# jhauret/vibravox

Measured on AMD Instinct MI355X. Metric: EBEN train-step audio-seconds/sec (gen+disc), higher is better.
Workload: dtype bf16

## Files before the change

vibravox_amd/csrc/gen_conv.hip:

```cpp
#include "common.h"

#include <cstdlib>
#include <type_traits>

namespace eben {

typedef float f32x16 __attribute__((ext_vector_type(16)));
typedef float f32x2 __attribute__((ext_vector_type(2)));
typedef __bf16 bf16x8 __attribute__((ext_vector_type(8)));
typedef __bf16 bf16x2 __attribute__((ext_vector_type(2)));
typedef unsigned u32x4 __attribute__((ext_vector_type(4)));

struct GcArgs {
  const float* x; float* y; const u32x4* wp; const float* bias; const float* res;
  int B, CX, LX, CY, LY, NU, S;
  int rpc_shift, off0, KSP, nkg;
  int nrt, nrg, ncb, nh;
  int reflect;
  float in_slope, out_slope, res_slope;
  long long w_rt, w_half;
  unsigned xq, xr;
};

__device__ __forceinline__ unsigned gc_pack2(float a, float b) {
// ... 267 lines not shown
        __syncthreads();
      }
    };
    for (int ch = 0; ch + 1 < nch; ++ch) chunk(ch, std::true_type{});
    chunk(nch - 1, std::false_type{});
  };
  bool allfast = true;
#pragma unroll
  for (int ct = 0; ct < CT; ++ct) allfast = allfast && fast[ct];
  if (allfast) {
    if (act_in) run(std::true_type{}, std::true_type{});
    else run(std::true_type{}, std::false_type{});
  } else {
    if (act_in) run(std::false_type{}, std::true_type{});
    else run(std::false_type{}, std::false_type{});
  }

  if (EBEN_GC_DBG & 8) {
    float s = 0.f;
#pragma unroll
    for (int ct = 0; ct < CT; ++ct)
#pragma unroll
      for (int i = 0; i < RT; ++i)
#pragma unroll
        for (int r = 0; r < 16; ++r) s += acc[ct][i][r];
    if (s == 1.2345f) P.y[0] = s;
    return;
  }
  float* yb = P.y + (long long)b * P.CY * P.LY;
  const float* rb = P.res ? P.res + (long long)b * P.CY * P.LY : nullptr;
#pragma unroll
  for (int ct = 0; ct < CT; ++ct) {
    const int u = u0w + ct * 32 + n;
    if (u >= P.NU) continue;
#pragma unroll
    for (int i = 0; i < RT; ++i) {
      const int mt = (rg * RT + i) * 32;
#pragma unroll
      for (int r4 = 0; r4 < 4; ++r4) {
        const int m = mt + 8 * r4 + 4 * hk;
        float o[4];
#pragma unroll
        for (int r = 0; r < 4; ++r) o[r] = acc[ct][i][4 * r4 + r];
        if (FORM != 2) {
#pragma unroll
          for (int r = 0; r < 4; ++r) {
            const float t = o[r] + (P.bias ? P.bias[m + r] : 0.f);
            const long long yi = (long long)(m + r) * P.LY + u;
            yb[yi] = lrelu(t, P.out_slope) + (rb ? lrelu(rb[yi], P.res_slope) : 0.f);
          }
        } else if (P.S == 8) {
          const int co = m >> 2;
          const float bv = P.bias ? P.bias[co] : 0.f;
          f32x4 t;
#pragma unroll
          for (int r = 0; r < 4; ++r) t[r] = lrelu(o[r] + bv, P.out_slope);
          const long long yi = (long long)co * P.LY + 8 * u + 4 * h;
          if (rb) {
            const f32x4 rv = *reinterpret_cast<const f32x4*>(rb + yi);
#pragma unroll
            for (int r = 0; r < 4; ++r) t[r] += lrelu(rv[r], P.res_slope);
          }
          *reinterpret_cast<f32x4*>(yb + yi) = t;
        } else if (P.S == 4) {
#pragma unroll
          for (int c2 = 0; c2 < 2; ++c2) {
            const int co = (m >> 1) + c2;
            const float bv = P.bias ? P.bias[co] : 0.f;
            f32x2 t;
            t[0] = lrelu(o[2 * c2] + bv, P.out_slope); t[1] = lrelu(o[2 * c2 + 1] + bv, P.out_slope);
            const long long yi = (long long)co * P.LY + 4 * u + 2 * h;
            if (rb) { t[0] += lrelu(rb[yi], P.res_slope); t[1] += lrelu(rb[yi + 1], P.res_slope); }
            *reinterpret_cast<f32x2*>(yb + yi) = t;
          }
        } else {
#pragma unroll
          for (int r = 0; r < 4; ++r) {
            const float t = o[r] + (P.bias ? P.bias[m + r] : 0.f);
            const long long yi = (long long)(m + r) * P.LY + 2 * u + h;
            yb[yi] = lrelu(t, P.out_slope) + (rb ? lrelu(rb[yi], P.res_slope) : 0.f);
          }
        }
      }
    }
  }
}

struct GcPackArgs {
  const float* w; const float* scale; u32x4* wp;
  int form, CX, CY, k, S, pad, rpc_shift, nkg, KSP, nrt, nh, np;
  long long total;
};

__global__ __launch_bounds__(256) void gc_pack_kernel(const GcPackArgs P) {
  const long long i = (long long)blockIdx.x * 256 + threadIdx.x;
  if (i >= P.total) return;
  const int lane = (int)(i & 63);
  long long r = i >> 6;
  const int q = (int)(r % P.np); r /= P.np;
  const int ks = (int)(r % P.KSP); r /= P.KSP;
  const int rt = (int)(r % P.nrt);
  const int h = (int)(r / P.nrt);
  const int mr = rt * 32 + (lane & 31);
  const int kg = 2 * ks + (lane >> 5);
  float v[8];
#pragma unroll
  for (int e = 0; e < 8; ++e) {
    float t = 0.f;
    if (kg < P.nkg) {
      if (P.form != 2) {
        const int chan = P.form == 0 ? kg >> P.rpc_shift : 2 * kg + (e >> 2);
        const int j = P.form == 0 ? 8 * (kg & ((1 << P.rpc_shift) - 1)) + e : (e & 3);
        if (j < P.k && chan < P.CX && mr < P.CY)
          t = P.w[((long long)mr * P.CX + chan) * P.k + j] * (P.scale ? P.scale[mr] : 1.f);
      } else {
        const int chan = 4 * kg + (e >> 1);
        const int hs = P.S >> 1;
        const int co = mr / hs, p = h * hs + mr % hs;
        const int du = h == 0 ? 1 - (e & 1) : -(e & 1);
        const int j = P.S * du + p + P.pad;
        if (j >= 0 && j < P.k && chan < P.CX && co < P.CY)
          t = P.w[((long long)chan * P.CY + co) * P.k + j] * (P.scale ? P.scale[chan] : 1.f);
      }
    }
    v[e] = t;
  }
  u32x4 o;
  for (int qq = 0;; ++qq) {
    o[0] = gc_pack2(v[0], v[1]); o[1] = gc_pack2(v[2], v[3]); o[2] = gc_pack2(v[4], v[5]); o[3] = gc_pack2(v[6], v[7]);
    if (qq == q) break;
#pragma unroll
    for (int u = 0; u < 4; ++u) {
      v[2 * u] -= __builtin_bit_cast(float, o[u] << 16);
      v[2 * u + 1] -= __builtin_bit_cast(float, o[u] & 0xffff0000u);
    }
  }
  P.wp[i] = o;
}

static int gc_env(const char* name, int dflt) {
  const char* s = getenv(name);
  return s ? atoi(s) : dflt;
}

struct GcPlan {
  int ok, form, np;
  int CX, LX, CY, LY, NU, S, k, pad, rpc_shift, nkg, KSP, rows, nrt, nh;
  int RT, CT, nrg, ncb;
};

static void gc_plan(const Canon& c, int dir, GcPlan* p) {
  static const int enabled = gc_env("EBEN_GC", 1);
  memset(p, 0, sizeof(*p));
  if (!enabled || c.bl || (c.np != 3 && c.np != 2) || c.g != 1 || c.d != 1 || c.xsplit_dir >= 0) return;
  p->np = c.np;
  p->S = c.s; p->k = c.k;
  if (dir == 0) {
    const bool enc = c.k == 2 * c.s && (c.s == 2 || c.s == 4 || c.s == 8);
    const bool lat = c.s == 1 && c.k >= 5 && c.k <= 8;
    if (!(enc || lat) || c.Cin % 16 || c.Cout % 32) return;
    if (c.reflect && (c.pl > c.Lin - 1 || c.pr > c.Lin - 1)) return;
    p->form = c.k <= 4 ? 1 : 0;
    p->CX = c.Cin; p->LX = c.Lin; p->CY = c.Cout; p->LY = c.Lout; p->NU = c.Lout;
    p->pad = c.pl;
    p->rpc_shift = c.k > 8 ? 1 : 0;
    p->nkg = p->form == 0 ? c.Cin << p->rpc_shift : c.Cin / 2;
    p->rows = c.Cout; p->nh = 1;
  } else {
    if (c.s != 2 && c.s != 4 && c.s != 8) return;
    if (c.k != 2 * c.s || c.pl != c.s / 2 || c.Lin != c.s * c.Lout) return;
    if (c.Cout % 16 || (c.Cin * (c.s / 2)) % 32) return;
    p->form = 2;
    p->CX = c.Cout; p->LX = c.Lout; p->CY = c.Cin; p->LY = c.Lin; p->NU = c.Lout;
    p->pad = c.pl;
    p->nkg = c.Cout / 4;
    p->rows = c.Cin * (c.s / 2); p->nh = 2;
  }
  p->KSP = round_up(ceil_div(p->nkg, 2), 8);
  p->nrt = p->rows / 32;
  static const int env_rt = gc_env("EBEN_GC_RT", 0), env_ct = gc_env("EBEN_GC_CT", 0);
  double best = 1e30;
  const int prod = p->np == 3 ? 6 : p->np == 2 ? 3 : 1;
  for (int rt : {2, 1}) {
    if (p->nrt % rt) continue;
    for (int ct : {2, 1}) {
      if (rt == 1 && ct == 2) continue;
      if ((env_rt && rt != env_rt && p->nrt % env_rt == 0) || (env_ct && ct != env_ct)) continue;
      const int ncb = ceil_div(p->NU, 128 * ct);
      const long long waves = 4ll * p->nh * (p->nrt / rt) * c.B * ncb;
      const double per_wave = (double)p->KSP * ct * (32.0 * prod * rt > 240.0 ? 32.0 * prod * rt : 240.0) + 2500.0 + 600.0 * rt * ct;
      const double t = (double)((waves + 1023) / 1024) * per_wave * (ct == 2 ? 1.05 : 1.0);
      if (t < best * 0.98) { best = t; p->RT = rt; p->CT = ct; }
    }
  }
  if (!p->RT) return;
  p->nrg = p->nrt / p->RT;
  p->ncb = ceil_div(p->NU, 128 * p->CT);
  p->ok = 1;
}

int gc_applicable(const Canon& c, int dir) {
  GcPlan p;
  gc_plan(c, dir, &p);
  return p.ok;
}

size_t gc_packed_floats(const Canon& c, int dir) {
  GcPlan p;
  gc_plan(c, dir, &p);
  return p.ok ? (size_t)p.nh * p.nrt * p.KSP * p.np * 64 * 4 : 0;
}

int gc_pack(const Canon& c, int dir, const float* w, const float* scale, float* wp, hipStream_t st) {
  GcPlan p;
  gc_plan(c, dir, &p);
  if (!p.ok) return fail(EBEN_EUNSUPPORTED, "gc_pack on a layer the direct-operand conv does not cover");
  GcPackArgs a{};
  a.w = w; a.scale = scale; a.wp = reinterpret_cast<u32x4*>(wp);
  a.form = p.form; a.CX = p.CX; a.CY = p.CY; a.k = p.k; a.S = p.S; a.pad = p.pad; a.rpc_shift = p.rpc_shift; a.nkg = p.nkg; a.KSP = p.KSP;
  a.nrt = p.nrt; a.nh = p.nh; a.np = p.np;
  a.total = (long long)p.nh * p.nrt * p.KSP * p.np * 64;
  hipLaunchKernelGGL(gc_pack_kernel, dim3((unsigned)((a.total + 255) / 256)), dim3(256), 0, st, a);
  EBEN_CHECK_LAUNCH("gc_pack_kernel");
  return EBEN_OK;
}

template <int FORM, int NP>
static void gc_launch_shape(const GcPlan& p, const GcArgs& a, unsigned grid, hipStream_t st) {
  if (p.RT == 2 && p.CT == 2) hipLaunchKernelGGL((gc_kernel<FORM, 2, 2, NP>), dim3(grid), dim3(256), 0, st, a);
  else if (p.RT == 2) hipLaunchKernelGGL((gc_kernel<FORM, 2, 1, NP>), dim3(grid), dim3(256), 0, st, a);
  else hipLaunchKernelGGL((gc_kernel<FORM, 1, 1, NP>), dim3(grid), dim3(256), 0, st, a);
}

int gc_launch(const Canon& c, int dir, const TapIO& io, hipStream_t st) {
  GcPlan p;
  gc_plan(c, dir, &p);
  if (!p.ok) return fail(EBEN_EUNSUPPORTED, "gc_launch on a layer the direct-operand conv does not cover");
  if (io.emask || io.in_mode || io.accumulate || io.res_rows || io.fm_sums) return fail(EBEN_EUNSUPPORTED, "direct-operand conv: forward launches only");
  GcArgs a{};
  a.x = io.x; a.y = io.y; a.wp = reinterpret_cast<const u32x4*>(io.wp); a.bias = io.bias; a.res = io.res;
  a.B = c.B; a.CX = p.CX; a.LX = p.LX; a.CY = p.CY; a.LY = p.LY; a.NU = p.NU; a.S = p.S;
  a.rpc_shift = p.rpc_shift; a.off0 = -p.pad; a.KSP = p.KSP; a.nkg = p.nkg;
  a.nrt = p.nrt; a.nrg = p.nrg; a.ncb = p.ncb; a.nh = p.nh;
  a.reflect = dir == 0 ? c.reflect : 0;
  a.in_slope = io.in_slope; a.out_slope = io.out_slope; a.res_slope = io.res_slope;
  a.w_rt = (long long)p.KSP * p.np * 64; a.w_half = a.w_rt * p.nrt;
  const unsigned grid = (unsigned)(p.nh * p.nrg * c.B * p.ncb);
  a.xq = grid / 8; a.xr = grid % 8;
  if (p.np == 2) {
    if (p.form == 0) gc_launch_shape<0, 2>(p, a, grid, st);
    else if (p.form == 1) gc_launch_shape<1, 2>(p, a, grid, st);
    else gc_launch_shape<2, 2>(p, a, grid, st);
  } else if (p.form == 0) gc_launch_shape<0, 3>(p, a, grid, st);
  else if (p.form == 1) gc_launch_shape<1, 3>(p, a, grid, st);
  else gc_launch_shape<2, 3>(p, a, grid, st);
  EBEN_CHECK_LAUNCH("gc_kernel");
  return EBEN_OK;
}

}
```

vibravox_amd/csrc/ru_split.hip:

```cpp
#include "common.h"

#include <cstdlib>

namespace eben {

#ifndef EBEN_RU_DBG
#define EBEN_RU_DBG 0
#endif

typedef float f32x16 __attribute__((ext_vector_type(16)));
typedef float f32x2 __attribute__((ext_vector_type(2)));
typedef __bf16 bf16x8 __attribute__((ext_vector_type(8)));
typedef __bf16 bf16x2 __attribute__((ext_vector_type(2)));
typedef unsigned u32x4 __attribute__((ext_vector_type(4)));

__device__ __forceinline__ unsigned rs_pack_bf16(float a, float b) {
  const f32x2 v = {a, b};
  return __builtin_bit_cast(unsigned, __builtin_convertvector(v, bf16x2));
}

template <int NP>
__device__ __forceinline__ void rs_split8(const float (&v)[8], u32x4 (&p)[NP]) {
  float r[8];
#pragma unroll
// ... 170 lines not shown
        for (int q = 0; q < 4; ++q) {
          uint2 v;
          v.x = rs_pack_bf16(acc1[i][4 * q], acc1[i][4 * q + 1]);
          v.y = rs_pack_bf16(acc1[i][4 * q + 2], acc1[i][4 * q + 3]);
          if (!(EBEN_RU_DBG & 2) || v.x == 0x12345u) hu[(long long)(4 * i + q) * L * 2] = v;
        }
    }
  } else if (P.h != nullptr && live) {
    float* __restrict__ hb = P.h + lbase;
#pragma unroll
    for (int i = 0; i < CT; ++i)
#pragma unroll
      for (int r = 0; r < 16; ++r) {
        const unsigned m = i * 32 + (r & 3) + 8 * (r >> 2) + 4 * (lane >> 5);
        hb[m * (unsigned)L] = acc1[i][r];
      }
  }

#pragma unroll
  for (int c2 = 0; c2 < NCH2; ++c2) {
    const int ch = NCH1 + c2;
    if (ch + 1 < NCHK) issue_w(ch + 1);
    const u32x4* wb = Ws + (ch & 1) * WCHU + lane;
#pragma unroll
    for (int kk = 0; kk < KSC; ++kk) {
      const int ks2 = c2 * KSC + kk;
      const int isrc = ks2 >> 1, s = ks2 & 1;
      float v[8];
#pragma unroll
      for (int e = 0; e < 8; ++e) v[e] = acc1[isrc][8 * s + e];
      u32x4 a[NP][CT], bq[NP];
#pragma unroll
      for (int q = 0; q < NP; ++q)
#pragma unroll
        for (int i = 0; i < CT; ++i) a[q][i] = wb[kk * U + (q * CT + i) * 64];
      rs_split8<NP>(v, bq);
      rs_mma<NP, CT>(a, bq, acc2);
    }
    if (c2 + 1 < NCH2) __syncthreads();
  }

  if constexpr (BL) {
    unsigned nlo = 0, nhi = 0;
#pragma unroll
    for (int i = 0; i < CT; ++i)
#pragma unroll
      for (int q = 0; q < 4; ++q) {
        unsigned nib = 0;
#pragma unroll
        for (int e = 0; e < 4; ++e) nib |= (acc2[i][4 * q + e] > 0.f ? 1u : 0u) << e;
        if (i < 2) nlo |= nib << (4 * (4 * i + q));
        else nhi |= nib << (4 * (4 * (i - 2) + q));
      }
    const unsigned olo = __shfl_xor(nlo, 32, 64), ohi = CT > 2 ? __shfl_xor(nhi, 32, 64) : 0u;
    const int hf = lane >> 5;
    const unsigned l0 = hf ? olo : nlo, l1 = hf ? nlo : olo, h0 = hf ? ohi : nhi, h1 = hf ? nhi : ohi;
    if (live) {
      unsigned char* __restrict__ ub8 = P.um + ubase;
#pragma unroll
      for (int g = 0; g < 4 * CT; g += 2) {
        const int gg = g + hf;
        const unsigned w0 = gg < 8 ? l0 : h0, w1 = gg < 8 ? l1 : h1;
        const int sh = 4 * (gg & 7);
        ub8[(long long)gg * L] = (unsigned char)(((w0 >> sh) & 15u) | (((w1 >> sh) & 15u) << 4));
      }
    }
  }

  if (!live) return;
  const float* xc = Xs + xshift + d + col;
  float* __restrict__ yb = P.y + lbase;
  float* __restrict__ ub = P.u + lbase;
  const bool keep_u = !BL && P.u != nullptr;
#pragma unroll
  for (int i = 0; i < CT; ++i)
#pragma unroll
    for (int r = 0; r < 16; ++r) {
      const unsigned m = i * 32 + (r & 3) + 8 * (r >> 2) + 4 * (lane >> 5);
      const unsigned off = m * (unsigned)L;
      const float uu = lrelu(acc2[i][r], P.out_slope);
      if (keep_u) ub[off] = uu;
      if (!(EBEN_RU_DBG & 1) || uu == 12345.f) yb[off] = xc[m * XS] + uu;
    }
}

__device__ __forceinline__ void ru3_pack_fwd_body(const float* __restrict__ vd, const float* __restrict__ sd, const float* __restrict__ vp,
                                                  const float* __restrict__ sp, u32x4* __restrict__ img, int CT, int NP, unsigned bid, unsigned nblk) {
  const int C = 32 * CT, KB = C / 16;
  const int total = 4 * KB * CT * 64;
  for (int t = bid * 256 + threadIdx.x; t < total; t += nblk * 256) {
    const int lane = t & 63;
    const int i = (t >> 6) % CT;
    const int ks = t / (64 * CT);
    const int m = 32 * i + (lane & 31), kh = lane >> 5;
    float w[8];
    if (ks < 3 * KB) {
      const int j = ks / KB, cb = ks - j * KB;
#pragma unroll
      for (int e = 0; e < 8; ++e) w[e] = vd[((long long)m * C + cb * 16 + 8 * kh + e) * 3 + j] * (sd ? sd[m] : 1.f);
    } else {
      const int ks2 = ks - 3 * KB, isrc = ks2 >> 1, s = ks2 & 1;
#pragma unroll
      for (int e = 0; e < 8; ++e) {
        const int chn = 32 * isrc + (e & 3) + 8 * (2 * s + (e >> 2)) + 4 * kh;
        w[e] = vp[(long long)m * C + chn] * (sp ? sp[m] : 1.f);
      }
    }
    float r[8];
#pragma unroll
    for (int e = 0; e < 8; ++e) r[e] = w[e];
    for (int q = 0; q < NP; ++q) {
      u32x4 o;
#pragma unroll
      for (int e = 0; e < 4; ++e) o[e] = rs_pack_bf16(r[2 * e], r[2 * e + 1]);
      img[((long long)(ks * NP + q) * CT + i) * 64 + lane] = o;
#pragma unroll
      for (int e = 0; e < 4; ++e) {
        r[2 * e] -= __builtin_bit_cast(float, o[e] << 16);
        r[2 * e + 1] -= __builtin_bit_cast(float, o[e] & 0xffff0000u);
      }
    }
  }
}

struct Ru3BwdArgs {
  const float* gy; const float* u; const u32x4* wimg; const float* xmask; const float* post; float* gx; float* gh;
  int B, L, d, ntt, BO, vec;
  float out_slope, in_slope;
};

template <int CT, int NW, int NP, int G>
__global__ __launch_bounds__(NW * 64, (NW == 4 && CT < 4) ? 2 : 1) void ru3_bwd_kernel(const Ru3BwdArgs P) {
  constexpr int NT = NW * 64, WN = NW * 32, C = 32 * CT;
  constexpr int GS = WN + 4;
  constexpr int U = NP * CT * 64;
  constexpr int EU = 2 * U;
  constexpr int WCHU = G * EU;
  static_assert(CT % G == 0, "an entry group never straddles a stage");

  extern __shared__ __attribute__((aligned(16))) u32x4 rs_smem[];
  u32x4* Ws = rs_smem;
  float* Gs = reinterpret_cast<float*>(rs_smem + 2 * WCHU);

  const int tid = threadIdx.x, lane = tid & 63;
  const int wn = __builtin_amdgcn_readfirstlane(tid >> 6);
  const int tt = __builtin_amdgcn_readfirstlane(blockIdx.x % P.ntt);
  const int b = __builtin_amdgcn_readfirstlane(blockIdx.x / P.ntt);
  const int d = P.d, L = P.L, BO = P.BO;
  const int t0 = tt * BO;
  const int w0 = t0 - d;
  const int wa = w0 >= 0 ? (w0 & ~3) : w0;
  const int xshift = w0 - wa;
  const long long rowbase = (long long)b * C * L;

  const bool fold_l = t0 <= d && L > 1;
  const bool fold_r = t0 + BO > L - 1 - d && t0 <= L - 2;
  const int NS = 4 * CT + (fold_l ? CT : 0) + (fold_r ? CT : 0);
  const int NSG = NS / G;
  auto img_entry = [&](int sq) -> int {
    if (sq < 4 * CT) return sq;
    sq -= 4 * CT;
    if (fold_l) { if (sq < CT) return CT + 2 * CT + sq; sq -= CT; }
    return CT + sq;
  };
  auto issue_w = [&](int sg) {
    u32x4* dst = Ws + (sg & 1) * WCHU;
// ... 182 lines not shown

__device__ __forceinline__ void ru3_pack_bwd_body(const float* __restrict__ vd, const float* __restrict__ sd, const float* __restrict__ vp,
                                                  const float* __restrict__ sp, u32x4* __restrict__ img, int CT, int NP, unsigned bid, unsigned nblk) {
  const int C = 32 * CT;
  const int total = 4 * CT * 2 * CT * 64;
  for (int t = bid * 256 + threadIdx.x; t < total; t += nblk * 256) {
    const int lane = t & 63;
    const int i = (t >> 6) % CT;
    const int kk = (t / (64 * CT)) & 1;
    const int en = t / (128 * CT);
    const int row = 32 * i + (lane & 31), kh = lane >> 5;
    float w[8];
#pragma unroll
    for (int e = 0; e < 8; ++e) {
      if (en < CT) {
        const int m = en * 32 + kk * 16 + 8 * kh + e;
        w[e] = vp[(long long)m * C + row] * (sp ? sp[m] : 1.f);
      } else {
        const int jj = (en - CT) / CT, cb = (en - CT) - jj * CT;
        const int m = cb * 32 + kk * 16 + 8 * kh + e;
        w[e] = vd[((long long)m * C + row) * 3 + (2 - jj)] * (sd ? sd[m] : 1.f);
      }
    }
    float r[8];
#pragma unroll
    for (int e = 0; e < 8; ++e) r[e] = w[e];
    for (int q = 0; q < NP; ++q) {
      u32x4 o;
#pragma unroll
      for (int e = 0; e < 4; ++e) o[e] = rs_pack_bf16(r[2 * e], r[2 * e + 1]);
      img[(((long long)(en * 2 + kk) * NP + q) * CT + i) * 64 + lane] = o;
#pragma unroll
      for (int e = 0; e < 4; ++e) {
        r[2 * e] -= __builtin_bit_cast(float, o[e] << 16);
        r[2 * e + 1] -= __builtin_bit_cast(float, o[e] & 0xffff0000u);
      }
    }
  }
}

__global__ __launch_bounds__(256) void ru3_pack_fwd_kernel(const float* vd, const float* sd, const float* vp, const float* sp, u32x4* img, int CT, int NP) {
  ru3_pack_fwd_body(vd, sd, vp, sp, img, CT, NP, blockIdx.x, gridDim.x);
}
__global__ __launch_bounds__(256) void ru3_pack_bwd_kernel(const float* vd, const float* sd, const float* vp, const float* sp, u32x4* img, int CT, int NP) {
  ru3_pack_bwd_body(vd, sd, vp, sp, img, CT, NP, blockIdx.x, gridDim.x);
}

constexpr int RU_PACK_MULTI = 48;
struct RuPackTable {
  int n;
  unsigned short first[RU_PACK_MULTI + 1];
  struct { const float* vd; const float* sd; const float* vp; const float* sp; u32x4* img; short CT, NP, which, pad; } job[RU_PACK_MULTI];
};
__global__ __launch_bounds__(256) void ru3_pack_multi_kernel(const RuPackTable T) {
  int j = 0;
#pragma unroll 1
  while (j + 1 < T.n && blockIdx.x >= T.first[j + 1]) ++j;
  const unsigned bid = blockIdx.x - T.first[j], nblk = T.first[j + 1] - T.first[j];
  if (T.job[j].which == 0) ru3_pack_fwd_body(T.job[j].vd, T.job[j].sd, T.job[j].vp, T.job[j].sp, T.job[j].img, T.job[j].CT, T.job[j].NP, bid, nblk);
  else ru3_pack_bwd_body(T.job[j].vd, T.job[j].sd, T.job[j].vp, T.job[j].sp, T.job[j].img, T.job[j].CT, T.job[j].NP, bid, nblk);
}

static int rs_pieces(int math) {
  switch (math) {
    case EBEN_MATH_BF16: return 1;
    case EBEN_MATH_BF16X3: return 2;
    case EBEN_MATH_BF16X6: return 3;
    default: return 0;
  }
}

template <int CT, int NW, int NP, int KSC, bool BL = false>
static int launch_ru3_fwd(const Ru3Args& a, hipStream_t st) {
  static LdsAttrOnce attr_once;
  auto kern = ru3_fwd_kernel<CT, NW, NP, KSC, BL>;
  constexpr int XS = NW * 32 + 2 * RS_DMAX + 6;
  const size_t lds = (size_t)2 * KSC * NP * CT * 64 * 16 + sizeof(float) * 32 * CT * XS;
  {
    const hipError_t e = lds_attr_once(attr_once, reinterpret_cast<const void*>(kern));
    if (e != hipSuccess) return hip_fail(e, "hipFuncSetAttribute(ru3_fwd)");
  }
  hipLaunchKernelGGL(kern, dim3(a.B * a.ntt), dim3(NW * 64), lds, st, a);
  EBEN_CHECK_LAUNCH("ru3_fwd_kernel");
  return EBEN_OK;
}

template <int CT, int NW, int NP, int G>
static int launch_ru3_bwd(const Ru3BwdArgs& a, hipStream_t st) {
  static LdsAttrOnce attr_once;
  auto kern = ru3_bwd_kernel<CT, NW, NP, G>;
  constexpr int GS = NW * 32 + 4;
  const size_t lds = (size_t)2 * G * 2 * NP * CT * 64 * 16 + sizeof(float) * 32 * CT * GS;
  {
    const hipError_t e = lds_attr_once(attr_once, reinterpret_cast<const void*>(kern));
    if (e != hipSuccess) return hip_fail(e, "hipFuncSetAttribute(ru3_bwd)");
  }
  hipLaunchKernelGGL(kern, dim3(a.B * a.ntt), dim3(NW * 64), lds, st, a);
  EBEN_CHECK_LAUNCH("ru3_bwd_kernel");
  return EBEN_OK;
}

static int rs_waves(int channels) {
  static const int w128 = getenv("EBEN_RU3_W128") ? atoi(getenv("EBEN_RU3_W128")) : 4;
  return channels == 128 ? (w128 == 4 ? 4 : 2) : 4;
}

int ru3_supported(int channels, int dilation, int math) {
  return (channels == 32 || channels == 64 || channels == 128) && dilation >= 1 && dilation <= RS_DMAX && rs_pieces(math) > 0;
}

size_t ru3_packed_floats(int channels, int math) {
  const int np = rs_pieces(math);
  if (np == 0 || (channels != 32 && channels != 64 && channels != 128)) return 0;
  return (size_t)2 * np * channels * channels;
}

int ru3_pack(int channels, int math, int which, const float* vd, const float* sd, const float* vp, const float* sp, float* wimg, hipStream_t st) {
  const int np = rs_pieces(math), CT = channels / 32;
  const int total = which == 0 ? 8 * CT * CT * 64 : 4 * CT * 2 * CT * 64;
  if (which == 0)
    hipLaunchKernelGGL(ru3_pack_fwd_kernel, dim3(ceil_div(total, 256)), dim3(256), 0, st, vd, sd, vp, sp, reinterpret_cast<u32x4*>(wimg), CT, np);
  else
    hipLaunchKernelGGL(ru3_pack_bwd_kernel, dim3(ceil_div(total, 256)), dim3(256), 0, st, vd, sd, vp, sp, reinterpret_cast<u32x4*>(wimg), CT, np);
  EBEN_CHECK_LAUNCH("ru3_pack_kernel");
  return EBEN_OK;
}

int ru3_fwd(int math, int batch, int channels, int length, int dilation, const float* x, float in_slope, float out_slope, const float* wimg,
            float* y, float* h, float* u, hipStream_t st) {
  Ru3Args a;
  a.x = x; a.wimg = reinterpret_cast<const u32x4*>(wimg); a.y = y; a.h = h; a.u = u;
  a.xb = nullptr; a.hb = nullptr; a.um = nullptr;
  a.B = batch; a.L = length; a.d = dilation;
  const int bn = rs_waves(channels) * 32;
  a.ntt = ceil_div(length, bn);
  a.in_slope = in_slope; a.out_slope = out_slope;
  a.vec = ((reinterpret_cast<uintptr_t>(x) & 15) == 0 && (length & 3) == 0) ? 1 : 0;
  if ((long long)a.B * a.ntt > 0x7fffffffLL) return fail(EBEN_EINVAL, "ResidualUnit grid too large");
  const int np = rs_pieces(math);
#define EBEN_RU3_FWD(NPV)                                                 \
  switch (channels / 32) {                                                \
    case 1: return launch_ru3_fwd<1, 4, NPV, 2>(a, st);                   \
    case 2: return launch_ru3_fwd<2, 4, NPV, 2>(a, st);                   \
    default: return rs_waves(128) == 4 ? launch_ru3_fwd<4, 4, NPV, 2>(a, st) : launch_ru3_fwd<4, 2, NPV, 1>(a, st); \
  }
  switch (np) {
    case 1: EBEN_RU3_FWD(1)
    case 2: EBEN_RU3_FWD(2)
    default: EBEN_RU3_FWD(3)
  }
#undef EBEN_RU3_FWD
}

int ru3_fwd_bl(int math, int batch, int channels, int length, int dilation, const float* x, float in_slope, float out_slope, const float* wimg,
               float* y, void* xb, void* hb, void* um, hipStream_t st) {
  Ru3Args a;
  a.x = x; a.wimg = reinterpret_cast<const u32x4*>(wimg); a.y = y; a.h = nullptr; a.u = nullptr;
  a.xb = static_cast<u32x4*>(xb); a.hb = static_cast<u32x4*>(hb); a.um = static_cast<unsigned char*>(um);
  a.B = batch; a.L = length; a.d = dilation;
  a.ntt = ceil_div(length, 128);
  a.in_slope = in_slope; a.out_slope = out_slope;
  a.vec = ((reinterpret_cast<uintptr_t>(x) & 15) == 0 && (length & 3) == 0) ? 1 : 0;
  if ((long long)a.B * a.ntt > 0x7fffffffLL) return fail(EBEN_EINVAL, "ResidualUnit grid too large");
  const int np = rs_pieces(math);
  if (np != 3 && np != 2) return fail(EBEN_EUNSUPPORTED, "eben_rubl_fwd: the forward computes in EBEN_MATH_BF16X6 or EBEN_MATH_BF16X3 (got %d)", math);
  if (np == 2) {
    switch (channels / 32) {
      case 1: return launch_ru3_fwd<1, 4, 2, 2, true>(a, st);
      case 2: return launch_ru3_fwd<2, 4, 2, 2, true>(a, st);
      default: return launch_ru3_fwd<4, 4, 2, 2, true>(a, st);
    }
  }
  switch (channels / 32) {
    case 1: return launch_ru3_fwd<1, 4, 3, 2, true>(a, st);
    case 2: return launch_ru3_fwd<2, 4, 3, 2, true>(a, st);
    default: return launch_ru3_fwd<4, 4, 3, 2, true>(a, st);
  }
}

int ru3_bwd(int math, int batch, int channels, int length, int dilation, const float* gy, const float* u, float out_slope, const float* x,
            float in_slope, const float* post, const float* wimg, float* gx, float* gh, hipStream_t st) {
  Ru3BwdArgs a;
  a.gy = gy; a.u = u; a.wimg = reinterpret_cast<const u32x4*>(wimg); a.xmask = in_slope != 1.f ? x : nullptr; a.post = post; a.gx = gx; a.gh = gh;
  a.B = batch; a.L = length; a.d = dilation;
  const int nw = rs_waves(channels);
  const int wn = nw * 32;
  a.BO = wn - 2 * dilation; a.ntt = ceil_div(length, a.BO);
  a.out_slope = out_slope; a.in_slope = in_slope;
  a.vec = (((reinterpret_cast<uintptr_t>(gy) | reinterpret_cast<uintptr_t>(u)) & 15) == 0 && (length & 3) == 0) ? 1 : 0;
  if ((long long)a.B * a.ntt > 0x7fffffffLL) return fail(EBEN_EINVAL, "ResidualUnit grid too large");
  const int np = rs_pieces(math);
  switch (np) {
    case 1:
      switch (channels / 32) {
        case 1: return launch_ru3_bwd<1, 4, 1, 1>(a, st);
        case 2: return launch_ru3_bwd<2, 4, 1, 2>(a, st);
        default: return nw == 4 ? launch_ru3_bwd<4, 4, 1, 2>(a, st) : launch_ru3_bwd<4, 2, 1, 2>(a, st);
      }
    case 2:
      switch (channels / 32) {
        case 1: return launch_ru3_bwd<1, 4, 2, 1>(a, st);
        case 2: return launch_ru3_bwd<2, 4, 2, 2>(a, st);
        default: return rs_waves(128) == 4 ? launch_ru3_bwd<4, 4, 2, 1>(a, st) : launch_ru3_bwd<4, 2, 2, 1>(a, st);
      }
    default:
      switch (channels / 32) {
        case 1: return launch_ru3_bwd<1, 4, 3, 1>(a, st);
        case 2: return launch_ru3_bwd<2, 4, 3, 1>(a, st);
        default: return rs_waves(128) == 4 ? launch_ru3_bwd<4, 4, 3, 1>(a, st) : launch_ru3_bwd<4, 2, 3, 1>(a, st);
      }
  }
}

}

using namespace eben;

extern "C" size_t eben_ru_packed_floats_ex(int channels, int math) {
  if (math == EBEN_MATH_F32) return eben_ru_packed_floats(channels);
  return ru3_packed_floats(channels, math);
}

extern "C" int eben_ru_supported(int channels, int dilation, int math) {
  if (math == EBEN_MATH_F32) return (channels == 32 || channels == 64 || channels == 128) && dilation >= 1 && dilation <= 16;
  return ru3_supported(channels, dilation, math);
}

extern "C" int eben_ru_pack_ex(int channels, int math, int which, const float* v_dil, const float* scale_dil, const float* v_pw,
                               const float* scale_pw, float* wimg, void* stream) {
  EBEN_REQUIRE(which == 0 || which == 1, "ru_pack_ex: which = 0 (forward image) or 1 (backward image)");
  if (math == EBEN_MATH_F32)
    return which == 0 ? eben_ru_pack(channels, v_dil, scale_dil, v_pw, scale_pw, wimg, stream)
                      : eben_ru_pack_bwd(channels, v_dil, scale_dil, v_pw, scale_pw, wimg, stream);
  EBEN_REQUIRE(ru3_supported(channels, 1, math), "fused ResidualUnit: 32, 64 or 128 channels and a known math mode (got %d, %d)", channels, math);
  EBEN_REQUIRE(v_dil && v_pw && wimg, "null pointer in ru_pack_ex");
  return ru3_pack(channels, math, which, v_dil, scale_dil, v_pw, scale_pw, wimg, as_stream(stream));
}

extern "C" int eben_ru_pack_multi(const EbenRuPackJob* jobs, int n, void* stream) {
  EBEN_REQUIRE(n >= 0 && (n == 0 || jobs != nullptr), "bad ru pack job list");
  for (int base = 0; base < n; base += RU_PACK_MULTI) {
    RuPackTable T;
    T.n = n - base < RU_PACK_MULTI ? n - base : RU_PACK_MULTI;
    T.first[0] = 0;
    for (int j = 0; j < T.n; ++j) {
      const EbenRuPackJob& jb = jobs[base + j];
      EBEN_REQUIRE(jb.math != EBEN_MATH_F32, "ru_pack_multi: the split-operand images only (pack the fp32 MFMA images with eben_ru_pack)");
      EBEN_REQUIRE(ru3_supported(jb.channels, 1, jb.math) && (jb.which == 0 || jb.which == 1) && jb.v_dil && jb.v_pw && jb.wimg, "bad ru pack job %d", base + j);
// ... 42 lines not shown
```

Before: 7437.

## Add split-K gen conv kernel for small grids and presplit RU forward

Adds a split-K variant of the direct-operand generator conv. When the grid would be small (short outputs, deep K), four waves each take a quarter of the K steps and their partial sums are reduced through LDS, giving more blocks and waves on the GPU. It also adds a residual-unit forward kernel for the 2-piece bf16 path that splits the input into bf16 pieces once while staging it in LDS, so the split is not repeated per k-step. Both are on by default, with the presplit kernel limited to 128+ channels unless the env var is set to 2. The cost is extra LDS traffic, a block-level reduction and more code paths.

```diff
diff --git a/vibravox_amd/csrc/gen_conv.hip b/vibravox_amd/csrc/gen_conv.hip
--- a/vibravox_amd/csrc/gen_conv.hip
+++ b/vibravox_amd/csrc/gen_conv.hip
@@ -373,6 +373,160 @@
           }
         }
       }
+    }
+  }
+}
+
+template <int RT, int NP>
+__global__ __launch_bounds__(256, 2) void gc_ks_kernel(const GcArgs P) {
+  constexpr int KD = 4;
+  __shared__ __attribute__((aligned(16))) float Rs[4 * RT * 16 * 64];
+
+  const int tid = threadIdx.x;
+  const int lane = tid & 63;
+  const int wave = __builtin_amdgcn_readfirstlane(tid >> 6);
+  const int n = lane & 31, hk = lane >> 5;
+
+  unsigned id;
+  {
+    const unsigned bid = blockIdx.x, xcd = bid & 7u, idx = bid >> 3;
+    id = (xcd < P.xr ? xcd * (P.xq + 1) : P.xr * (P.xq + 1) + (xcd - P.xr) * P.xq) + idx;
+  }
+  const int rg = __builtin_amdgcn_readfirstlane((int)(id % (unsigned)P.nrg)); id /= (unsigned)P.nrg;
+  const int cb = __builtin_amdgcn_readfirstlane((int)(id % (unsigned)P.ncb));
+  const int b = __builtin_amdgcn_readfirstlane((int)(id / (unsigned)P.ncb));
+
+  const float* xb = P.x + (long long)b * P.CX * P.LX;
+  const u32x4* wsrc = P.wp + (long long)(rg * RT) * P.w_rt;
+  const int nk = P.KSP >> 2, ks0 = wave * nk;
+
+  typedef const __attribute__((address_space(1))) char* gptr_t;
+  const int u0 = cb * 32;
+  const int ucol = u0 + n < P.NU ? u0 + n : P.NU - 1;
+  const bool fast = u0 + 31 < P.NU && P.S * u0 + P.off0 >= 0 && P.S * (u0 + 31) + P.off0 + (8 << P.rpc_shift) <= P.LX;
+  const bool act_in = P.in_slope != 1.f;
+  const int ks_real = P.nkg >> 1;
+  const int RKS = P.rpc_shift ? 1 : 2;
+  const int loff = (P.rpc_shift ? 8 * hk : hk * P.LX) + P.S * ucol + P.off0;
+  auto row_ptr = [&](int ks) -> gptr_t {
+    const int kc = ks < ks_real ? ks : ks_real - 1;
+    unsigned long long a = reinterpret_cast<unsigned long long>(xb + (long long)(kc * RKS) * P.LX);
+    asm volatile("" : "+s"(a));
+    return reinterpret_cast<gptr_t>(a);
+  };
+  auto w_ptr = [&](int ks) -> gptr_t {
+    unsigned long long a = reinterpret_cast<unsigned long long>(wsrc + (long long)ks * (NP * 64));
+    asm volatile("" : "+s"(a));
+    return reinterpret_cast<gptr_t>(a);
+  };
+  struct Slow { int off[8]; unsigned ok; };
+  Slow sl;
+  if (!fast) {
+    sl.ok = 0;
+#pragma unroll
+    for (int e = 0; e < 8; ++e) {
+      const int crow = P.rpc_shift ? 0 : hk;
+      int pos = P.S * ucol + P.off0 + (P.rpc_shift ? 8 * hk : 0) + e;
+      if (P.reflect) {
+        pos = pos < 0 ? -pos : pos;
+        pos = pos >= P.LX ? 2 * (P.LX - 1) - pos : pos;
+      }
+      const bool ok = pos >= 0 && pos < P.LX;
+      sl.off[e] = crow * P.LX + (ok ? pos : 0);
+      sl.ok |= (unsigned)ok << e;
+    }
+  }
+
+  f32x16 acc[RT];
+#pragma unroll
+  for (int i = 0; i < RT; ++i)
+#pragma unroll
+    for (int r = 0; r < 16; ++r) acc[i][r] = 0.f;
+
+  auto run = [&](auto fast_tag, auto act_tag) {
+    constexpr bool FAST = decltype(fast_tag)::value;
+    float v[KD][8];
+    u32x4 aq[KD][NP][RT];
+    typedef float f4u __attribute__((ext_vector_type(4), aligned(4)));
+    typedef const __attribute__((address_space(1))) f4u* g4_t;
+    typedef const __attribute__((address_space(1))) float* g1_t;
+    typedef const __attribute__((address_space(1))) u32x4* gu_t;
+    auto ask = [&](int k, int s) {
+      const int ks = ks0 + (k < nk ? k : nk - 1);
+      const gptr_t rp = row_ptr(ks);
+      if constexpr (FAST) {
+        const unsigned o = (unsigned)loff * 4u;
+        const f4u a0 = *reinterpret_cast<g4_t>(rp + o), a1 = *reinterpret_cast<g4_t>(rp + 16 + o);
+#pragma unroll
+        for (int e = 0; e < 4; ++e) { v[s][e] = a0[e]; v[s][4 + e] = a1[e]; }
+      } else {
+#pragma unroll
+        for (int e = 0; e < 8; ++e) v[s][e] = *reinterpret_cast<g1_t>(rp + (unsigned)sl.off[e] * 4u);
+      }
+      const gptr_t wq = w_ptr(ks);
+#pragma unroll
+      for (int q = 0; q < NP; ++q)
+#pragma unroll
+        for (int i = 0; i < RT; ++i)
+          aq[s][q][i] = *reinterpret_cast<gu_t>(wq + ((unsigned)i * (unsigned)P.w_rt + (unsigned)(q * 64 + lane)) * 16u);
+    };
+#pragma unroll
+    for (int s = 0; s < KD; ++s) ask(s, s);
+    for (int k = 0; k < nk; k += KD) {
+#pragma unroll
+      for (int s = 0; s < KD; ++s) {
+        if constexpr (!FAST) {
+#pragma unroll
+          for (int e = 0; e < 8; ++e) v[s][e] = (sl.ok >> e) & 1u ? v[s][e] : 0.f;
+        }
+        if constexpr (decltype(act_tag)::value) {
+#pragma unroll
+          for (int e = 0; e < 8; ++e) v[s][e] = lrelu(v[s][e], P.in_slope);
+        }
+        u32x4 bq[NP];
+        gc_split<NP>(v[s], bq);
+#pragma unroll
+        for (int lvl = NP - 1; lvl >= 0; --lvl)
+#pragma unroll
+          for (int qw = 0; qw < NP; ++qw) {
+            const int qx = lvl - qw;
+            if (qx < 0 || qx >= NP) continue;
+#pragma unroll
+            for (int i = 0; i < RT; ++i)
+              acc[i] = __builtin_amdgcn_mfma_f32_32x32x16_bf16(__builtin_bit_cast(bf16x8, aq[s][qw][i]), __builtin_bit_cast(bf16x8, bq[qx]), acc[i], 0, 0, 0);
+          }
+        ask(k + s + KD, s);
+        __builtin_amdgcn_sched_barrier(0);
+      }
+    }
+  };
+  if (fast) {
+    if (act_in) run(std::true_type{}, std::true_type{});
+    else run(std::true_type{}, std::false_type{});
+  } else {
+    if (act_in) run(std::false_type{}, std::true_type{});
+    else run(std::false_type{}, std::false_type{});
+  }
+
+#pragma unroll
+  for (int i = 0; i < RT; ++i)
+#pragma unroll
+    for (int r = 0; r < 16; ++r) Rs[((wave * RT + i) * 16 + r) * 64 + lane] = acc[i][r];
+  __syncthreads();
+  const int u = u0 + n;
+  if (u >= P.NU) return;
+  float* yb = P.y + (long long)b * P.CY * P.LY;
+  const float* rb = P.res ? P.res + (long long)b * P.CY * P.LY : nullptr;
+#pragma unroll
+  for (int i = 0; i < RT; ++i) {
+    const int m = (rg * RT + i) * 32 + 8 * wave + 4 * hk;
+#pragma unroll
+    for (int r = 0; r < 4; ++r) {
+      const int ri = (i * 16 + 4 * wave + r) * 64 + lane;
+      const float o = (Rs[ri] + Rs[RT * 1024 + ri]) + (Rs[2 * RT * 1024 + ri] + Rs[3 * RT * 1024 + ri]);
+      const float t = o + (P.bias ? P.bias[m + r] : 0.f);
+      const long long yi = (long long)(m + r) * P.LY + u;
+      yb[yi] = lrelu(t, P.out_slope) + (rb ? lrelu(rb[yi], P.res_slope) : 0.f);
     }
   }
 }
@@ -438,6 +592,7 @@
   int ok, form, np;
   int CX, LX, CY, LY, NU, S, k, pad, rpc_shift, nkg, KSP, rows, nrt, nh;
   int RT, CT, nrg, ncb;
+  int ksplit;
 };
 
 static void gc_plan(const Canon& c, int dir, GcPlan* p) {
@@ -488,6 +643,21 @@
   p->nrg = p->nrt / p->RT;
   p->ncb = ceil_div(p->NU, 128 * p->CT);
   p->ok = 1;
+  static const int ksplit = gc_env("EBEN_GC_KSPLIT", 1);
+  if (ksplit && p->form == 0 && p->NU <= 128 && p->KSP >= 64 && p->KSP % 16 == 0 && (long long)p->nh * p->nrg * c.B * p->ncb < 128) {
+    const int ncb = ceil_div(p->NU, 32);
+    double bt = 1e30;
+    int brt = 0;
+    for (int rt : {2, 1}) {
+      if (p->nrt % rt) continue;
+      const long long waves = 4ll * (p->nrt / rt) * c.B * ncb;
+      const double per_wave = (double)(p->KSP / 4) * (32.0 * prod * rt > 240.0 ? 32.0 * prod * rt : 240.0) + 2500.0 + 600.0 * rt;
+      const double t = (double)((waves + 1023) / 1024) * per_wave;
+      if (t < bt * 0.98) { bt = t; brt = rt; }
+    }
+    p->ksplit = 1; p->RT = brt; p->CT = 1;
+    p->nrg = p->nrt / brt; p->ncb = ncb;
+  }
 }
 
 int gc_applicable(const Canon& c, int dir) {
@@ -538,6 +708,15 @@
   a.w_rt = (long long)p.KSP * p.np * 64; a.w_half = a.w_rt * p.nrt;
   const unsigned grid = (unsigned)(p.nh * p.nrg * c.B * p.ncb);
   a.xq = grid / 8; a.xr = grid % 8;
+  if (p.ksplit) {
+    if (p.np == 2) {
+      if (p.RT == 2) hipLaunchKernelGGL((gc_ks_kernel<2, 2>), dim3(grid), dim3(256), 0, st, a);
+      else hipLaunchKernelGGL((gc_ks_kernel<1, 2>), dim3(grid), dim3(256), 0, st, a);
+    } else if (p.RT == 2) hipLaunchKernelGGL((gc_ks_kernel<2, 3>), dim3(grid), dim3(256), 0, st, a);
+    else hipLaunchKernelGGL((gc_ks_kernel<1, 3>), dim3(grid), dim3(256), 0, st, a);
+    EBEN_CHECK_LAUNCH("gc_ks_kernel");
+    return EBEN_OK;
+  }
   if (p.np == 2) {
     if (p.form == 0) gc_launch_shape<0, 2>(p, a, grid, st);
     else if (p.form == 1) gc_launch_shape<1, 2>(p, a, grid, st);
diff --git a/vibravox_amd/csrc/ru_split.hip b/vibravox_amd/csrc/ru_split.hip
--- a/vibravox_amd/csrc/ru_split.hip
+++ b/vibravox_amd/csrc/ru_split.hip
@@ -276,6 +276,228 @@
       if (keep_u) ub[off] = uu;
       if (!(EBEN_RU_DBG & 1) || uu == 12345.f) yb[off] = xc[m * XS] + uu;
     }
+}
+
+template <int CT, int KSC>
+__global__ __launch_bounds__(256, CT < 4 ? 2 : 1) void ru3_fwd_ps_kernel(const Ru3Args P) {
+  constexpr int NP = 2, NT = 256, BN = 128, C = 32 * CT;
+  constexpr int XS = BN + 2 * RS_DMAX + 6;
+  constexpr int PS = (C / 8) * XS;
+  constexpr int KB = C / 16;
+  constexpr int KS1 = 3 * KB, KS2 = KB;
+  constexpr int U = NP * CT * 64;
+  constexpr int WCHU = KSC * U;
+  constexpr int NCH1 = KS1 / KSC, NCH2 = KS2 / KSC, NCHK = NCH1 + NCH2;
+  static_assert(KS1 % KSC == 0 && KS2 % KSC == 0, "a chunk never straddles the two stages");
+  static_assert(KSC % 2 == 0, "the fragment registers alternate by k-step and start every chunk at 0");
+  static_assert(XS % 4 == 0 && WCHU % 64 == 0, "four positions per staging item, chunks are whole wave pieces");
+
+  extern __shared__ __attribute__((aligned(16))) u32x4 rs_smem[];
+  u32x4* Ws = rs_smem;
+  u32x4* Xp = rs_smem + 2 * WCHU;
+
+  const int tid = threadIdx.x, lane = tid & 63;
+  const int wn = __builtin_amdgcn_readfirstlane(tid >> 6);
+  const int tt = __builtin_amdgcn_readfirstlane(blockIdx.x % P.ntt);
+  const int b = __builtin_amdgcn_readfirstlane(blockIdx.x / P.ntt);
+  const int t0 = tt * BN, d = P.d, L = P.L;
+  const int q0 = t0 - d;
+  const int qa = q0 >= 0 ? (q0 & ~3) : q0;
+  const int xshift = q0 - qa;
+  const float* xrow = P.x + (long long)b * C * L;
+
+  auto issue_w = [&](int ch) {
+    const u32x4* src = P.wimg + (long long)ch * WCHU;
+    u32x4* dst = Ws + (ch & 1) * WCHU;
+#pragma unroll
+    for (int p = 0; p * NT < WCHU; ++p) {
+      const int idx = p * NT + tid;
+      if (idx < WCHU)
+        __builtin_amdgcn_global_load_lds((const __attribute__((address_space(1))) void*)(src + idx),
+                                         (__attribute__((address_space(3))) void*)(dst + (idx & ~63)), 16, 0, 0);
+    }
+  };
+  issue_w(0);
+
+  const bool interior = P.vec && q0 >= 0 && qa + XS <= L;
+  if (interior) {
+    constexpr int x4 = XS >> 2, tot = (C / 8) * x4;
+    for (int base = 0; base < tot; base += NT) {
+      const int i = base + tid;
+      if (i < tot) {
+        const int g = i / x4;
+        const int k4 = i - g * x4;
+        const float* src = xrow + (long long)(8 * g) * L + qa + 4 * k4;
+        f32x4 v[8];
+#pragma unroll
+        for (int e = 0; e < 8; ++e) v[e] = *reinterpret_cast<const f32x4*>(src + (unsigned)e * (unsigned)L);
+        u32x4* dst = Xp + g * XS + 4 * k4;
+#pragma unroll
+        for (int p = 0; p < 4; ++p) {
+          float t[8];
+#pragma unroll
+          for (int e = 0; e < 8; ++e) t[e] = lrelu(v[e][p], P.in_slope);
+          u32x4 pc[NP];
+          rs_split8<NP>(t, pc);
+#pragma unroll
+          for (int q = 0; q < NP; ++q) dst[q * PS + p] = pc[q];
+        }
+      }
+    }
+  } else {
+    constexpr int tot = (C / 8) * XS;
+    for (int base = 0; base < tot; base += NT) {
+      const int i = base + tid;
+      if (i < tot) {
+        const int g = i / XS;
+        const int p = i - g * XS;
+        int q = qa + p;
+        q = q < 0 ? -q : q;
+        q = q >= L ? 2 * (L - 1) - q : q;
+        const bool ok = q >= 0 && q < L;
+        const float* src = xrow + (long long)(8 * g) * L + (ok ? q : 0);
+        float t[8];
+#pragma unroll
+        for (int e = 0; e < 8; ++e) t[e] = src[(unsigned)e * (unsigned)L];
+#pragma unroll
+        for (int e = 0; e < 8; ++e) t[e] = ok ? lrelu(t[e], P.in_slope) : 0.f;
+        u32x4 pc[NP];
+        rs_split8<NP>(t, pc);
+#pragma unroll
+        for (int q2 = 0; q2 < NP; ++q2) Xp[q2 * PS + g * XS + p] = pc[q2];
+      }
+    }
+  }
+
+  f32x16 acc1[CT], acc2[CT];
+#pragma unroll
+  for (int i = 0; i < CT; ++i)
+#pragma unroll
+    for (int r = 0; r < 16; ++r) { acc1[i][r] = 0.f; acc2[i][r] = 0.f; }
+
+  const int col = wn * 32 + (lane & 31);
+  const int hf = lane >> 5;
+  const u32x4* xu = Xp + hf * XS + xshift + col;
+  const int t = t0 + col;
+  const bool live = t < L;
+  const long long ubase = (long long)b * (C / 8) * L + t;
+
+  u32x4 a[2][NP][CT], bq[2][NP];
+  auto read_a = [&](int ch, int kk, u32x4 (&af)[NP][CT]) {
+    const u32x4* wb = Ws + (ch & 1) * WCHU + kk * U + lane;
+#pragma unroll
+    for (int q = 0; q < NP; ++q)
+#pragma unroll
+      for (int i = 0; i < CT; ++i) af[q][i] = wb[(q * CT + i) * 64];
+  };
+  auto read_b = [&](int ks, u32x4 (&bf)[NP]) {
+    const int j = ks / KB, cb = ks - j * KB;
+    const u32x4* xk = xu + 2 * cb * XS + j * d;
+#pragma unroll
+    for (int q = 0; q < NP; ++q) bf[q] = xk[q * PS];
+  };
+
+  __syncthreads();
+  issue_w(1);
+  read_a(0, 0, a[0]);
+  read_b(0, bq[0]);
+
+#pragma nounroll
+  for (int ch = 0; ch < NCH1; ++ch) {
+#pragma unroll
+    for (int kk = 0; kk < KSC; ++kk) {
+      const int ks = ch * KSC + kk;
+      if (kk + 1 < KSC) {
+        read_a(ch, kk + 1, a[(kk + 1) & 1]);
+        read_b(ks + 1, bq[(kk + 1) & 1]);
+      } else {
+        __syncthreads();
+        if (ch + 2 < NCHK) issue_w(ch + 2);
+        read_a(ch + 1, 0, a[0]);
+        if (ks + 1 < KS1) read_b(ks + 1, bq[0]);
+      }
+      if (ks / KB == 1 && live) P.xb[ubase + (long long)(2 * (ks - KB) + hf) * L] = bq[kk & 1][0];
+      rs_mma<NP, CT>(a[kk & 1], bq[kk & 1], acc1);
+    }
+  }
+
+  if (live) {
+    uint2* __restrict__ hu = reinterpret_cast<uint2*>(P.hb + ubase) + hf;
+#pragma unroll
+    for (int i = 0; i < CT; ++i)
+#pragma unroll
+      for (int q = 0; q < 4; ++q) {
+        uint2 v;
+        v.x = rs_pack_bf16(acc1[i][4 * q], acc1[i][4 * q + 1]);
+        v.y = rs_pack_bf16(acc1[i][4 * q + 2], acc1[i][4 * q + 3]);
+        hu[(long long)(4 * i + q) * L * 2] = v;
+      }
+  }
+  float xin[CT][16];
+  const unsigned loff = (unsigned)(live ? t : L - 1) + 4u * (unsigned)hf * (unsigned)L;
+  {
+    const float* __restrict__ xc = xrow;
+#pragma unroll
+    for (int i = 0; i < CT; ++i)
+#pragma unroll
+      for (int r = 0; r < 16; ++r) xin[i][r] = xc[(unsigned)(i * 32 + (r & 3) + 8 * (r >> 2)) * (unsigned)L + loff];
+  }
+
+#pragma unroll
+  for (int c2 = 0; c2 < NCH2; ++c2) {
+    const int ch = NCH1 + c2;
+#pragma unroll
+    for (int kk = 0; kk < KSC; ++kk) {
+      const int ks2 = c2 * KSC + kk;
+      const int isrc = ks2 >> 1, s = ks2 & 1;
+      float v[8];
+#pragma unroll
+      for (int e = 0; e < 8; ++e) v[e] = acc1[isrc][8 * s + e];
+      u32x4 bs[NP];
+      rs_split8<NP>(v, bs);
+      if (kk + 1 < KSC) read_a(ch, kk + 1, a[(kk + 1) & 1]);
+      else if (c2 + 1 < NCH2) {
+        __syncthreads();
+        if (ch + 2 < NCHK) issue_w(ch + 2);
+        read_a(ch + 1, 0, a[0]);
+      }
+      rs_mma<NP, CT>(a[kk & 1], bs, acc2);
+    }
+  }
+
+  {
+    unsigned nlo = 0, nhi = 0;
+#pragma unroll
+    for (int i = 0; i < CT; ++i)
+#pragma unroll
+      for (int q = 0; q < 4; ++q) {
+        unsigned nib = 0;
+#pragma unroll
+        for (int e = 0; e < 4; ++e) nib |= (acc2[i][4 * q + e] > 0.f ? 1u : 0u) << e;
+        if (i < 2) nlo |= nib << (4 * (4 * i + q));
+        else nhi |= nib << (4 * (4 * (i - 2) + q));
+      }
+    const unsigned olo = __shfl_xor(nlo, 32, 64), ohi = CT > 2 ? __shfl_xor(nhi, 32, 64) : 0u;
+    const unsigned l0 = hf ? olo : nlo, l1 = hf ? nlo : olo, h0 = hf ? ohi : nhi, h1 = hf ? nhi : ohi;
+    if (live) {
+      unsigned char* __restrict__ ub8 = P.um + ubase;
+#pragma unroll
+      for (int g = 0; g < 4 * CT; g += 2) {
+        const int gg = g + hf;
+        const unsigned w0 = gg < 8 ? l0 : h0, w1 = gg < 8 ? l1 : h1;
+        const int sh = 4 * (gg & 7);
+        ub8[(long long)gg * L] = (unsigned char)(((w0 >> sh) & 15u) | (((w1 >> sh) & 15u) << 4));
+      }
+    }
+  }
+
+  if (!live) return;
+  float* __restrict__ yb = P.y + (long long)b * C * L;
+#pragma unroll
+  for (int i = 0; i < CT; ++i)
+#pragma unroll
+    for (int r = 0; r < 16; ++r)
+      yb[(unsigned)(i * 32 + (r & 3) + 8 * (r >> 2)) * (unsigned)L + loff] = lrelu(xin[i][r], P.in_slope) + lrelu(acc2[i][r], P.out_slope);
 }
 
 __device__ __forceinline__ void ru3_pack_fwd_body(const float* __restrict__ vd, const float* __restrict__ sd, const float* __restrict__ vp,
@@ -624,6 +846,21 @@
   }
   hipLaunchKernelGGL(kern, dim3(a.B * a.ntt), dim3(NW * 64), lds, st, a);
   EBEN_CHECK_LAUNCH("ru3_fwd_kernel");
+  return EBEN_OK;
+}
+
+template <int CT, int KSC>
+static int launch_ru3_fwd_ps(const Ru3Args& a, hipStream_t st) {
+  static LdsAttrOnce attr_once;
+  auto kern = ru3_fwd_ps_kernel<CT, KSC>;
+  constexpr int XS = 4 * 32 + 2 * RS_DMAX + 6;
+  const size_t lds = (size_t)2 * KSC * 2 * CT * 64 * 16 + (size_t)2 * (32 * CT / 8) * XS * 16;
+  {
+    const hipError_t e = lds_attr_once(attr_once, reinterpret_cast<const void*>(kern));
+    if (e != hipSuccess) return hip_fail(e, "hipFuncSetAttribute(ru3_fwd_ps)");
+  }
+  hipLaunchKernelGGL(kern, dim3(a.B * a.ntt), dim3(256), lds, st, a);
+  EBEN_CHECK_LAUNCH("ru3_fwd_ps_kernel");
   return EBEN_OK;
 }
 
@@ -706,6 +943,14 @@
   if ((long long)a.B * a.ntt > 0x7fffffffLL) return fail(EBEN_EINVAL, "ResidualUnit grid too large");
   const int np = rs_pieces(math);
   if (np != 3 && np != 2) return fail(EBEN_EUNSUPPORTED, "eben_rubl_fwd: the forward computes in EBEN_MATH_BF16X6 or EBEN_MATH_BF16X3 (got %d)", math);
+  static const int presplit = getenv("EBEN_RU_FWD_PRESPLIT") ? atoi(getenv("EBEN_RU_FWD_PRESPLIT")) : 1;
+  if (np == 2 && presplit) {
+    switch (channels / 32) {
+      case 1: if (presplit == 2) return launch_ru3_fwd_ps<1, 2>(a, st); break;
+      case 2: if (presplit == 2) return launch_ru3_fwd_ps<2, 2>(a, st); break;
+      default: return launch_ru3_fwd_ps<4, 2>(a, st);
+    }
+  }
   if (np == 2) {
     switch (channels / 32) {
       case 1: return launch_ru3_fwd<1, 4, 2, 2, true>(a, st);
```

Result: no change. 7427, median of 2 (-0.1%).
